# koesterlab/microphaser

Hardware: AMD Instinct MI355X
Metric: peptide-windows/s (somatic, 9-mer) (higher is better)
Workload: dtype u64

## Files before the change

### microphaser_amd/csrc/kernels.hip

```cpp
#include <hip/hip_runtime.h>

#include <algorithm>
#include <cstdlib>
#include <type_traits>

#include "kernels.hpp"

namespace mp {

#ifndef MP_KPART
#define MP_KPART -1
#endif
#define MP_IN_PART(n) (MP_KPART == -1 || MP_KPART == (n))
#define HIP_CHECK_LAUNCH() \
    do { hipError_t e_ = hipGetLastError(); if (e_ != hipSuccess) { throw_hip(e_, __FILE__, __LINE__); } } while (0)

[[noreturn]] void throw_hip(hipError_t e, const char* file, int line);

#if MP_IN_PART(0)
__global__ __launch_bounds__(256) void k0_read_variants(DeviceBatch d) {
    const uint32_t i = blockIdx.x * 256u + threadIdx.x;
    if (i >= d.n_reads) return;
    uint32_t lo = 0, hi = d.n_genes;
    while (hi - lo > 1) {
// ... 1916 lines not shown
                    tkey[idx] = 0ull;
                    tcnt[idx] = 0;
                }
                ng += uint32_t(__popcll(m));
            }
            if (ng == 0) {
                if (lane == 0) { skey[0] = 0ull; scnt[0] = 0; }
                ng = 1;
            }
            if (lane == 0) ng_lds = 0;
            __syncthreads();
            uint32_t werr = sticky_err;
            if (chunk_pos + ng > chunk_end) {
                chunk_pos = wave_claim(gcur, K2N_GROUP_CHUNK, gpart_lo);
                chunk_end = chunk_pos + K2N_GROUP_CHUNK;
            }
            const bool can_write = chunk_end <= gpart_hi;
            if (!can_write) werr |= WD_GROUP_OVERFLOW;
            if (can_write && rec_pos + ng > rec_end) {
                const uint32_t want = max(uint32_t(REC_CHUNK), ng);
                rec_pos = wave_claim(rcur, want, rpart_lo);
                rec_end = rec_pos + want;
            }
            if (can_write && rec_pos + ng > rpart_hi) sticky_err |= WD_REC_OVERFLOW;
            const uint64_t gbase = chunk_pos;
            if (can_write) {
                for (uint32_t g0 = 0; g0 < ng; g0 += 64) {
                    const uint32_t g = g0 + lane;
                    if (g < ng) {
                        const unsigned long long key = skey[g];
                        uint32_t rank = 0;
                        for (uint32_t j = 0; j < ng; j++) rank += skey[j] < key ? 1u : 0u;
                        Group G; G.hap = key; G.count = scnt[g]; G.aux = 0;
                        d.groups[gbase + rank] = G;
                    }
                    k3_enqueue(d, part, g < ng, gbase + g, win, rec_pos + g < rpart_hi ? uint32_t(rec_pos + g) : 0xFFFFFFFFu);
                }
                rec_pos += ng;
                chunk_pos += ng;
                n_groups_tx += ng;
            }
            if (lane == 0) {
                WinDyn wd;
                wd.group_off = uint32_t(gbase);
                wd.ngroups = ng;
                wd.nrows = nrows;
                wd.flags = WD_DONE | werr;
                d.win_dyn[win] = wd;
            }
            __syncthreads();
        }
    }
    if (sticky_err) atomicOr(d.err, sticky_err);
}

__device__ __forceinline__ bool is_upper(uint8_t c) { return c >= 'A' && c <= 'Z'; }
__device__ __forceinline__ uint8_t to_lower(uint8_t c) { return is_upper(c) ? uint8_t(c + 32) : c; }
__device__ __forceinline__ uint8_t to_upper(uint8_t c) { return (c >= 'a' && c <= 'z') ? uint8_t(c - 32) : c; }
__device__ __forceinline__ uint32_t rol32(uint32_t x, int n) { return (x << n) | (x >> (32 - n)); }

__device__ __forceinline__ void append_wanted(const DeviceBatch& d, bool want, uint32_t rec_slot) {
    const uint64_t m = __ballot(want);
    if (!m) return;
    const uint32_t lane = threadIdx.x & 63;
    const uint32_t leader = uint32_t(__builtin_ctzll(m));
    const uint32_t part = (blockIdx.x + blockIdx.y) & (NPART - 1);
    unsigned long long base = 0;
    if (lane == leader) base = atomicAdd(d.cursors + part * 32 + 24, (unsigned long long)__popcll(m));
    const uint64_t b0 = (uint64_t(rdlane(uint32_t(base >> 32), leader)) << 32) | rdlane(uint32_t(base), leader);
    if (want) {
        const uint64_t off = b0 + lanes_below(m, lane);
        if (off < (1ull << d.rec_part_log2)) d.want_recs[(uint64_t(part) << d.rec_part_log2) + off] = rec_slot;
        else atomicOr(d.err, WD_REC_OVERFLOW);
    }
}

constexpr int K3_THREADS = 64;
constexpr int K3_REFCAP = 36;
template <int CAP> struct K3Cfg {
    static constexpr int SLOT_BYTES = K3_REFCAP + 2 * CAP;
    static constexpr int SLOT_DW = (SLOT_BYTES / 4) | 1;
};

template <bool BUF>
struct ShaStreamT {
    uint32_t h0, h1, h2, h3, h4;
    uint64_t q;
    uint32_t nq, widx, total;
    uint32_t* blk;
    __device__ __forceinline__ void init(uint32_t* b) {
        h0 = 0x67452301u; h1 = 0xEFCDAB89u; h2 = 0x98BADCFEu; h3 = 0x10325476u; h4 = 0xC3D2E1F0u;
        q = 0; nq = 0; widx = 0; total = 0; blk = b;
    }
    __device__ void compress(uint32_t off = 0) {
        uint32_t w[16];
#pragma unroll
        for (int i = 0; i < 16; i++) w[i] = blk[off + i];
        uint32_t a = h0, b = h1, c = h2, d = h3, e = h4;
#pragma unroll
        for (int i = 0; i < 80; i++) {
            uint32_t wi;
            if (i < 16) wi = w[i];
            else {
                wi = rol32(w[(i + 13) & 15] ^ w[(i + 8) & 15] ^ w[(i + 2) & 15] ^ w[i & 15], 1);
                w[i & 15] = wi;
            }
            uint32_t f, k;
            if (i < 20) { f = (b & c) | (~b & d); k = 0x5A827999u; }
            else if (i < 40) { f = b ^ c ^ d; k = 0x6ED9EBA1u; }
            else if (i < 60) { f = (b & c) | (b & d) | (c & d); k = 0x8F1BBCDCu; }
            else { f = b ^ c ^ d; k = 0xCA62C1D6u; }
            uint32_t t = rol32(a, 5) + f + e + k + wi;
            e = d; d = c; c = rol32(b, 30); b = a; a = t;
        }
        h0 += a; h1 += b; h2 += c; h3 += d; h4 += e;
    }
    __device__ __forceinline__ void feed(uint64_t v, uint32_t n) {
        q = (q << (8 * n)) | v;
        nq += n;
        total += n;
        if (nq >= 4) {
            nq -= 4;
            blk[widx++] = uint32_t(q >> (8 * nq));
            if constexpr (!BUF) { if (widx == 16) { compress(); widx = 0; } }
            if (nq >= 4) {
                nq -= 4;
                blk[widx++] = uint32_t(q >> (8 * nq));
                if constexpr (!BUF) { if (widx == 16) { compress(); widx = 0; } }
            }
        }
    }
    __device__ void feed_dec(uint32_t v) {
        const uint32_t hi = v / 100000u, lo = v - hi * 100000u;
        auto chunk = [&](uint32_t x, bool pad) {
            uint64_t txt = 0;
            uint32_t n = 0;
            const uint32_t dg[5] = {x / 10000u, (x / 1000u) % 10u, (x / 100u) % 10u, (x / 10u) % 10u, x % 10u};
#pragma unroll
            for (int k = 0; k < 5; k++)
                if (pad || n || dg[k] || k == 4) { txt = (txt << 8) | ('0' + dg[k]); n++; }
            feed(txt, n);
        };
        if (hi) { chunk(hi, false); chunk(lo, true); }
        else chunk(lo, false);
    }
    __device__ void finish() {
        const uint32_t bits = total * 8;
        feed(0x80, 1);
        if (nq) feed(0, 4 - nq);
        while ((widx & 15) != 14) feed(0, 4);
        feed(0, 4);
        feed(bits, 4);
    }
};

__device__ __forceinline__ bool stop_codon_at(const uint8_t* s, uint32_t c, bool fwd) {
    uint8_t a = s[c], b = s[c + 1], e = s[c + 2];
    if (fwd) return a == 'T' && ((b == 'G' && e == 'A') || (b == 'A' && (e == 'G' || e == 'A')));
    return (a == 'T' && b == 'C' && e == 'A') || (a == 'C' && b == 'T' && e == 'A') || (a == 'T' && b == 'T' && e == 'A');
}

constexpr uint32_t K3B_BUF_WORDS = 48;
__device__ __forceinline__ void fill_byte_text(uint64_t* byte_text, uint32_t n_threads) {
    for (uint32_t v = threadIdx.x; v < 256; v += n_threads) {
        uint64_t txt;
        uint32_t n;
        if (v >= 100) { txt = (uint64_t('0' + v / 100) << 16) | (uint64_t('0' + (v / 10) % 10) << 8) | ('0' + v % 10); n = 3; }
        else if (v >= 10) { txt = (uint64_t('0' + v / 10) << 8) | ('0' + v % 10); n = 2; }
        else { txt = '0' + v; n = 1; }
        txt = (txt << 16) | (uint64_t(',') << 8) | ' ';
        byte_text[v] = (txt << 8) | (n + 2);
    }
}
template <int SEQ_CAP>
__device__ __forceinline__ uint64_t haplotype_id60(const DeviceBatch& d, bool active, const uint32_t* sq, uint32_t seq_len, uint32_t id_off, uint32_t id_len,
                                                   const uint32_t* idw, uint32_t id_mis, uint32_t win_sso, uint32_t* blk, const uint64_t* byte_text) {
    auto feed_message = [&](auto& sh) {
        sh.feed('[', 1);
#pragma unroll
        for (uint32_t k0 = 0; k0 < uint32_t(SEQ_CAP); k0 += 4) {
            if (k0 >= seq_len) break;
            const uint32_t dw = sq[k0 >> 2];
#pragma unroll
            for (int b = 0; b < 4; b++) {
                const uint32_t k = k0 + b;
                if (k < seq_len) {
                    const uint64_t e = byte_text[(dw >> (8 * b)) & 0xFF];
                    uint64_t txt = e >> 8;
                    uint32_t n = uint32_t(e & 0xFF);
                    if (k + 1 >= seq_len) { txt >>= 16; n -= 2; }
                    sh.feed(txt, n);
                }
            }
        }
        sh.feed(']', 1);
#pragma unroll
        for (uint32_t k = 0; k < 20; k += 4) {
            if (k < id_len) {
                const uint32_t n = min(4u, id_len - k);
                const uint32_t le = __builtin_amdgcn_alignbyte(idw[k / 4 + 1], idw[k / 4], id_mis);
                const uint32_t be = __builtin_bswap32(le) >> (8 * (4 - n));
                sh.feed(be, n);
            }
        }
        for (uint32_t k = 20; k < id_len; k += 4) {
            uint64_t txt = 0;
            const uint32_t n = min(4u, id_len - k);
            for (uint32_t c = 0; c < n; c++) txt = (txt << 8) | d.str_pool[id_off + k + c];
            sh.feed(txt, n);
        }
        sh.feed_dec(win_sso);
        sh.finish();
    };
    uint32_t o0 = 0, o1 = 0;
    const bool fits = 5 * seq_len + id_len + 20 <= K3B_BUF_WORDS * 4;
    if (__ballot(active && !fits) == 0) {
        ShaStreamT<true> sh;
        sh.init(blk);
        if (active) feed_message(sh);
        const uint32_t nblk = active ? sh.widx >> 4 : 0u;
        const uint32_t maxblk = __ballot(nblk >= 3) ? 3u : __ballot(nblk >= 2) ? 2u : __ballot(nblk >= 1) ? 1u : 0u;
        for (uint32_t bk = 0; bk < maxblk; bk++)
            if (bk < nblk) sh.compress(bk * 16);
        o0 = sh.h0; o1 = sh.h1;
    } else if (active) {
        ShaStreamT<false> sh;
        sh.init(blk);
        feed_message(sh);
        o0 = sh.h0; o1 = sh.h1;
    }
    return (uint64_t(o0) << 28) | (uint64_t(o1) >> 4);
}

template <int SEQ_CAP, int LIST, int THREADS, int K3_ITEMS>
__global__ __launch_bounds__(THREADS, LIST != 1 ? 2 : 4) void k3_window_seq(DeviceBatch d) {
    constexpr int K3_THREADS = THREADS;
    constexpr bool LIST_A = LIST != 1;
    constexpr bool STOPSCAN = LIST >= 2;
    constexpr bool WALK = LIST == 3;
    constexpr int K3_SLOT_DW = LIST_A ? ((K3Cfg<SEQ_CAP>::SLOT_DW > int(K3B_BUF_WORDS + 1) ? K3Cfg<SEQ_CAP>::SLOT_DW : int(K3B_BUF_WORDS + 1)) | 1) : K3Cfg<SEQ_CAP>::SLOT_DW;
    __shared__ uint32_t lds_slots[K3_THREADS * K3_SLOT_DW];
    __shared__ uint64_t byte_text[LIST_A ? 256 : 1];
    if constexpr (LIST_A) { fill_byte_text(byte_text, K3_THREADS); __syncthreads(); }
    const uint32_t tid = threadIdx.x;
    const uint32_t lpart = blockIdx.y;
    const uint64_t part_size = 1ull << d.group_part_log2;
    const uint64_t n_slots = min((unsigned long long)d.cursors[lpart * 32 + (LIST == 0 ? 8 : LIST == 1 ? 12 : LIST == 2 ? 20 : 28)], (unsigned long long)part_size);
    struct K3In {
        bool in_list;
        uint64_t li;
        uint64_t g;
        uint32_t w, rec_pre;
        uint64_t hap;
        WinStatic ws;
        const uint8_t* wref;
        uint32_t mis;
        uint32_t refw[K3_REFCAP / 4];
        uint32_t cp[8], ci[8];
        uint32_t id_off, id_len, id_mis;
        uint32_t idw[6];
    };
    auto load_entry = [&](K3In& I, uint64_t tile) __attribute__((always_inline)) {
        const uint64_t li = tile * K3_THREADS + tid;
        I.li = li;
        const uint64_t lidx = li < part_size ? li : part_size - 1;
        const uint64_t lpos = (uint64_t(lpart) << d.group_part_log2) + ((LIST & 1) ? part_size - 1 - lidx : lidx) + (LIST >= 2 ? d.group_cap : 0ull);
        const uint4 item = d.k3_items[lpos];
        I.g = item.x; I.w = item.y; I.rec_pre = item.z;
    };
    auto load_window = [&](K3In& I) __attribute__((always_inline)) {
        I.in_list = I.li < n_slots;
        if (!I.in_list) { I.g = 0; I.w = 0xFFFFFFFFu; I.rec_pre = 0xFFFFFFFFu; }
        if (I.w != 0xFFFFFFFFu && I.w >= d.n_wins) { I.w = 0xFFFFFFFFu; I.g = 0; }
        if (I.g >= d.group_cap) I.g = 0;
        const uint4* bp = reinterpret_cast<const uint4*>(d.win_blobs + (I.w != 0xFFFFFFFFu ? I.w : 0u));
        uint4 q[8];
#pragma unroll
        for (int k = 0; k < 8; k++) q[k] = bp[k];
        I.hap = d.groups[I.g].hap;
        static_assert(sizeof(WinStatic) == 32 && K3_REFCAP == 36, "WinBlob unpacking");
        uint32_t wsw[8] = {q[0].x, q[0].y, q[0].z, q[0].w, q[1].x, q[1].y, q[1].z, q[1].w};
        __builtin_memcpy(&I.ws, wsw, 32);
        I.refw[0] = q[2].x; I.refw[1] = q[2].y; I.refw[2] = q[2].z; I.refw[3] = q[2].w; I.refw[4] = q[3].x; I.refw[5] = q[3].y; I.refw[6] = q[3].z; I.refw[7] = q[3].w;
        I.refw[8] = q[4].x;
        const uint32_t cw[12] = {q[4].z, q[4].w, q[5].x, q[5].y, q[5].z, q[5].w, q[6].x, q[6].y, q[6].z, q[6].w, q[7].x, q[7].y};
#pragma unroll
        for (int k = 0; k < int(WINBLOB_COLS); k++) { I.cp[k] = cw[2 * k]; I.ci[k] = cw[2 * k + 1]; }
        I.id_off = q[7].z; I.id_len = q[7].w;
    };
    auto load_payload = [&](K3In& I) __attribute__((always_inline)) {
        const WinStatic& ws = I.ws;
        I.wref = d.ref_pool + ws.ref_off;
        I.mis = ws.ref_off & 3u;
        I.cp[6] = I.cp[7] = 0xFFFFFFFFu; I.ci[6] = I.ci[7] = 0;
        if (__ballot(I.w != 0xFFFFFFFFu && ws.ncols > WINBLOB_COLS)) {
            const uint32_t ncols = ws.ncols, last_c = ncols ? ncols - 1 : 0;
#pragma unroll
            for (uint32_t k = WINBLOB_COLS; k < 8; k++) { const WinCol* wc = d.win_cols + ws.col_off + min(k, last_c); I.cp[k] = wc->pos; I.ci[k] = wc->info; }
        }
    };
    auto load_id_text = [&](K3In& I) __attribute__((always_inline)) {
        I.id_mis = 0;
#pragma unroll
        for (int k = 0; k < 6; k++) I.idw[k] = 0;
        if constexpr (LIST_A) {
            const uint8_t* idp = d.str_pool + I.id_off;
            I.id_mis = uint32_t(reinterpret_cast<uintptr_t>(idp) & 3u);
#pragma unroll
            for (int k = 0; k < 6; k++) I.idw[k] = reinterpret_cast<const uint32_t*>(idp - I.id_mis)[k];
        }
    };
    uint32_t* const slot = lds_slots + tid * K3_SLOT_DW;
    uint8_t* const refb = reinterpret_cast<uint8_t*>(slot);
    uint8_t* const seq = refb + K3_REFCAP;
    uint8_t* const germ = seq + SEQ_CAP;
    auto process = [&](K3In& I) __attribute__((always_inline)) {
    const uint64_t g = I.g;
    const uint32_t w = I.w, rec_pre = I.rec_pre;
    const bool live = w != 0xFFFFFFFFu;
    const uint32_t id_off = I.id_off, id_len = I.id_len, id_mis = I.id_mis;
    const uint32_t* const idw = I.idw;
    uint32_t sumflags = 0;
    bool need_rec = false;
    uint64_t prof_set = 0;
    bool want_id = false;
    uint32_t seq_len = 0, germ_len = 0, prof_len = 0, nvar = 0, nsom = 0, first_fs = 0, first_fs_j = 0;
    uint32_t rec_sso = 0;
    if (live) {
        const WinStatic& ws = I.ws;
        rec_sso = ws.sso;
        const uint32_t vbase = ws.vbase;
        const uint64_t hap = I.hap;
        const bool is_rev = (ws.flags & WSF_REVERSE) != 0;
        const uint32_t ncols = ws.ncols;
        const uint32_t window_end = ws.sso + ws.wlen;
        const uint8_t* const wref = I.wref;
        const uint32_t mis = I.mis;
        const uint32_t* const cp = I.cp;
        const uint32_t* const ci = I.ci;
#pragma unroll
        for (int k = 0; k < K3_REFCAP / 4; k++) slot[k] = I.refw[k];
        const uint32_t staged = min(uint32_t(ws.wlen), uint32_t(K3_REFCAP) - mis);
        auto ref_at = [&](uint32_t pos) -> uint8_t {
            uint32_t k = pos - ws.sso;
            return k < staged ? refb[mis + k] : wref[k];
        };
        uint32_t i = ws.sso, j = 0, ns = 0, ngm = 0;
        bool indel = false, insertion = false, broke_flag = false;
        if (ws.flags & WSF_SIMPLE) {
#pragma unroll
            for (int k = 0; k < 8; k++) {
                const uint32_t v = __builtin_amdgcn_alignbyte(slot[k + 1], slot[k], mis);
                slot[K3_REFCAP / 4 + k] = v;
                slot[(K3_REFCAP + SEQ_CAP) / 4 + k] = v;
            }
            auto substitute = [&](uint32_t dq, uint32_t pos, uint32_t info) {
                const uint32_t off = pos - ws.sso;
                const uint8_t r = refb[mis + off];
                const uint8_t alt = uint8_t(info >> VI_ALT_SHIFT);
                const uint8_t sw = is_upper(r) ? to_lower(alt) : alt;
                seq[off] = sw;
                if (info & VI_GERMLINE) germ[off] = sw; else nsom++;
                nvar++;
                prof_set |= 1ull << (is_rev ? (ncols - 1 - dq) : dq);
            };
            const uint32_t vis = ws.need_recs >> WS_PREFIX_SHIFT;
            const uint32_t dlo = is_rev ? ncols - vis : 0u, dhi = is_rev ? ncols : vis;
#pragma unroll
            for (int k = 0; k < 8; k++)
                if (uint32_t(k) >= dlo && uint32_t(k) < dhi && ((hap >> (ncols - 1 - k)) & 1)) substitute(uint32_t(k), cp[k], ci[k]);
            for (uint32_t k = max(8u, dlo); k < dhi; k++)
                if ((hap >> (ncols - 1 - k)) & 1) { const WinCol wc = d.win_cols[ws.col_off + k]; substitute(k, wc.pos, wc.info); }
            ns = ngm = ws.wlen;
            j = vis;
            if (STOPSCAN && vis > 0 && vis < ncols) {
                const uint32_t dq_last = is_rev ? ncols - vis : vis - 1;
                const WinCol lc = d.win_cols[ws.col_off + dq_last];
                if (lc.pos + 1 == window_end && ((hap >> (ncols - 1 - dq_last)) & 1)) {
                    uint32_t cnt = 0;
                    for (uint32_t wi = vis; wi < ncols; wi++) {
                        const uint32_t dq = is_rev ? ncols - 1 - wi : wi;
                        const WinCol wc = d.win_cols[ws.col_off + dq];
                        if (wc.pos != window_end + cnt) break;
                        j = wi + 1;
                        if (!((hap >> (ncols - 1 - dq)) & 1)) break;
                        const uint32_t off = uint32_t(ws.wlen) + cnt;
                        const uint8_t r = ref_at(wc.pos);
                        const uint8_t alt = uint8_t(wc.info >> VI_ALT_SHIFT);
                        const uint8_t sw = is_upper(r) ? to_lower(alt) : alt;
                        if (off < uint32_t(SEQ_CAP)) { seq[off] = sw; germ[off] = (wc.info & VI_GERMLINE) ? sw : r; }
                        ns++; ngm++; cnt++;
                        if (!(wc.info & VI_GERMLINE)) nsom++;
                        nvar++;
                        prof_set |= 1ull << wi;
                    }
                }
            }
        } else if constexpr (!WALK) {
            atomicOr(d.err, WD_INTERNAL);
        } else {
            uint32_t pos_j = 0xFFFFFFFFu, info_j = 0, f_j = 0;
            uint32_t cpos[8], cinfo[8];
    #pragma unroll
            for (int k = 0; k < 8; k++) {
                cpos[k] = 0xFFFFFFFFu; cinfo[k] = 0;
                if (uint32_t(k) < ncols) {
                    const uint32_t dq = is_rev ? (ncols - 1 - k) : uint32_t(k);
                    if (is_rev || dq >= 8) { const WinCol* wc = d.win_cols + ws.col_off + dq; cpos[k] = wc->pos; cinfo[k] = wc->info; }
                    else { cpos[k] = cp[k]; cinfo[k] = ci[k]; }
                }
            }
            auto load_j = [&]() {
                if (j < 8) {
                    pos_j = cpos[0]; info_j = cinfo[0];
    #pragma unroll
                    for (int k = 1; k < 8; k++) if (j == uint32_t(k)) { pos_j = cpos[k]; info_j = cinfo[k]; }
                    if (j >= ncols) pos_j = 0xFFFFFFFFu;
                } else if (j < ncols) {
                    uint32_t dq = is_rev ? (ncols - 1 - j) : j;
                    const WinCol wc = d.win_cols[ws.col_off + dq];
                    pos_j = wc.pos;
                    info_j = wc.info;
                } else {
                    pos_j = 0xFFFFFFFFu;
                }
            };
            auto col_f = [&]() { return d.win_cols[ws.col_off + (is_rev ? (ncols - 1 - j) : j)].f; };
            auto push_s = [&](uint8_t c) { if (ns < SEQ_CAP) seq[ns] = c; ns++; };
            auto push_g = [&](uint8_t c) { if (ngm < SEQ_CAP) germ[ngm] = c; ngm++; };
            load_j();
            while (i < window_end) {
                while (j < ncols && i == pos_j) {
                    uint32_t fs = (info_j & VI_FS_MASK) >> VI_FS_SHIFT;
                    if (first_fs == 0 && fs) { first_fs = fs; first_fs_j = j; }
                    uint32_t dq = is_rev ? (ncols - 1 - j) : j;
                    uint32_t bit = ncols - 1 - dq;
                    if ((hap >> bit) & 1) {
// ... 4 lines not shown
                        if (kind == 0) {
                            uint8_t alt = uint8_t(info_j >> VI_ALT_SHIFT);
                            uint8_t sw = is_upper(r) ? to_lower(alt) : alt;
                            push_g(germline ? sw : r);
                            push_s(sw);
                            i += 1;
                        } else if (kind == 1) {
                            f_j = col_f();
                            uint32_t il = d.v_len[vbase + f_j] + 1;
                            const uint8_t* ins = d.ins_pool + d.v_insoff[vbase + f_j];
                            bool up = is_upper(r);
                            for (uint32_t k = 0; k < il; k++) {
                                uint8_t c = up ? to_lower(ins[k]) : to_upper(ins[k]);
                                if (germline) push_g(c);
                                push_s(c);
                            }
                            if (!germline) indel = true;
                            insertion = true;
                            i += 1;
                        } else {
                            f_j = col_f();
                            uint32_t dl = d.v_len[vbase + f_j];
                            if (is_rev && pos_j + dl - 1 >= window_end) { brk = true; }
                            else {
                                if (germline || i == window_end - 1) push_g(r);
                                else {
                                    for (uint32_t k = 0; k < dl + 1; k++) push_g(ref_at(i + k));
                                    indel = true;
                                }
                                push_s(r);
                                i += dl + 1;
                            }
                        }
                        if (brk) { broke_flag = true; break; }
                        if (!germline) nsom++;
                        nvar++;
                        prof_set |= 1ull << j;
                    }
                    j++;
                    load_j();
                }
                if (i < window_end) {
                    uint32_t stop_at = (j < ncols && pos_j > i) ? min(pos_j, window_end) : window_end;
                    for (; i < stop_at; i++) { uint8_t r = ref_at(i); push_s(r); push_g(r); }
                }
            }
        }
        seq_len = min(ns, uint32_t(SEQ_CAP));
        germ_len = min(ngm, uint32_t(SEQ_CAP));
        prof_len = j;
        uint32_t this_len = seq_len < ws.ewl ? seq_len : ws.ewl;
        uint32_t nlo = 0, nhi = seq_len;
        if (ws.splice_pos == 1) nlo = min(uint32_t(ws.splice_gap), seq_len);
        else if (ws.splice_pos == 0 && !insertion) nhi = this_len;
        bool stop = false;
        uint32_t nlen = nhi - nlo;
        if constexpr (!STOPSCAN) {
            if (!(ws.flags & WSF_NOSTOP)) atomicOr(d.err, WD_INTERNAL);
        } else if (nlen >= 3 && !(ws.flags & WSF_NOSTOP)) {
            if (!is_rev) {
                for (uint32_t c = 0; c + 3 <= nlen; c += 3)
                    if (stop_codon_at(seq + nlo, c, true)) { stop = true; break; }
            } else {
                for (int c = int(nlen) - 3; c >= 0; c -= 3)
                    if (stop_codon_at(seq + nlo, uint32_t(c), false)) { stop = true; break; }
            }
        }
        bool differs;
        if (!WALK || (ws.flags & WSF_SIMPLE)) differs = nsom > 0;
        else {
            differs = seq_len != germ_len;
            if (!differs)
                for (uint32_t k = 0; k < seq_len; k++)
                    if (seq[k] != germ[k]) { differs = true; break; }
        }
        sumflags = GS_VALID | (stop ? GS_STOP : 0) | (differs ? GS_DIFFERS : 0) | (indel ? GS_INDEL : 0) |
                   (insertion ? GS_INSERTION : 0) | (broke_flag ? GS_BROKE : 0);
        need_rec = nsom > 0 || (ws.need_recs & WS_MASK) != 0;
        want_id = need_rec && (nsom > 0 || (ws.need_recs & WS_ALL_IDS));
        if (stop && ws.splice_pos != 2 && !(ws.flags & SF_FIRST_EXON_WIN)) atomicMin(&d.tx_first_stop[ws.tx], w);
    }
    uint32_t recidx = 0;
    {
        uint32_t sqr[2 * SEQ_CAP / 4];
#pragma unroll
        for (int k = 0; k < 2 * SEQ_CAP / 4; k++) sqr[k] = slot[K3_REFCAP / 4 + k];
        const bool has_slot = live && rec_pre != 0xFFFFFFFFu;
        const bool hash = has_slot && need_rec && want_id;
        uint64_t id60 = 0;
        if constexpr (LIST_A) {
            id60 = haplotype_id60<SEQ_CAP>(d, hash && !d.timing_skip_ids, sqr, seq_len, id_off, id_len, idw, id_mis, rec_sso, slot, byte_text);
            const uint64_t hm = __ballot(hash);
            if (hm && (tid & 63u) == uint32_t(__builtin_ctzll(hm))) atomicAdd(d.cursors + ((blockIdx.x + blockIdx.y) & (NPART - 1)) * 32 + 24, (unsigned long long)__popcll(hm));
        } else if (hash) {
            atomicOr(d.err, WD_REC_OVERFLOW);
        }
        if (has_slot) {
            uint32_t* out = reinterpret_cast<uint32_t*>(d.recs + uint64_t(rec_pre) * d.rec_stride);
            if (need_rec) {
                uint4* const out4 = reinterpret_cast<uint4*>(out);
                out4[0] = make_uint4(uint32_t(prof_set), uint32_t(prof_set >> 32), uint32_t(id60), uint32_t(id60 >> 32));
                out4[1] = make_uint4(seq_len | (germ_len << 8) | (prof_len << 16) | (nvar << 24), nsom | (first_fs << 8) | (first_fs_j << 16), w, want_id ? 1u : 0u);
#pragma unroll
                for (int k = 0; k < SEQ_CAP / 16; k++) {
                    if (uint32_t(16 * k) < seq_len) out4[2 + k] = make_uint4(sqr[4 * k], sqr[4 * k + 1], sqr[4 * k + 2], sqr[4 * k + 3]);
                    if (uint32_t(16 * k) < germ_len) {
                        constexpr int G = SEQ_CAP / 16;
                        out4[2 + G + k] = make_uint4(sqr[4 * (G + k)], sqr[4 * (G + k) + 1], sqr[4 * (G + k) + 2], sqr[4 * (G + k) + 3]);
                    }
                }
                sumflags |= GS_HAS_REC | ((LIST_A && want_id) ? uint32_t(GS_ID_VALID) : 0u);
                recidx = rec_pre;
            } else {
                out[7] = 0;
            }
        } else if (live && need_rec) {
            atomicOr(d.err, WD_REC_OVERFLOW);
        }
    }
    if (live) {
        GroupSum gs;
        gs.flags = sumflags;
        gs.rec = recidx;
        d.gsum[g] = gs;
    }
    };
    for (uint64_t tile0 = uint64_t(blockIdx.x) * K3_ITEMS;; tile0 += uint64_t(gridDim.x) * K3_ITEMS) {
        static_assert(K3_ITEMS == 1 || K3_ITEMS == 2, "entries per lane");
        K3In in0, in1;
        load_entry(in0, tile0);
        if constexpr (K3_ITEMS == 2) load_entry(in1, tile0 + 1);
        if (tile0 * K3_THREADS >= n_slots) break;
        if (pass_overflowed(d)) return;
        load_window(in0);
        if constexpr (K3_ITEMS == 2) load_window(in1);
        load_payload(in0);
        if constexpr (K3_ITEMS == 2) load_payload(in1);
        load_id_text(in0);
        if constexpr (K3_ITEMS == 2) load_id_text(in1);
        process(in0);
        if constexpr (K3_ITEMS == 2) process(in1);
    }
}

template <int SEQ_CAP>
__device__ __forceinline__ uint32_t k3n_one(const DeviceBatch& d, uint32_t* lds_slots, uint64_t g, uint32_t item_win, uint32_t item_rec, bool valid,
                                            uint32_t& recidx) {
    constexpr int K3_SLOT_DW = K3Cfg<SEQ_CAP>::SLOT_DW;
    const uint32_t tid = threadIdx.x;
    recidx = 0;
    uint32_t* slot = lds_slots + tid * K3_SLOT_DW;
    uint8_t* refb = reinterpret_cast<uint8_t*>(slot);
    uint8_t* seq = refb + K3_REFCAP;
    uint32_t* germ_dw = slot + (K3_REFCAP + SEQ_CAP) / 4;
    const uint32_t w = valid ? item_win : 0xFFFFFFFFu;
    if (w == 0xFFFFFFFFu) return 0;
    const WinStatic ws = d.wins[w];
    const uint32_t vbase = ws.vbase;
    const Group G = d.groups[g];
    const uint64_t hap = G.hap;
    const uint32_t nrows = d.win_dyn[w].nrows;
    const bool freq_one = G.count != 0 && G.count == nrows;
    const bool is_rev = (ws.flags & WSF_REVERSE) != 0;
    const uint32_t ncols = ws.ncols;
    uint32_t window_end = ws.sso + ws.wlen;
    const uint8_t* wref = d.ref_pool + ws.ref_off;
    const uint32_t mis = uint32_t(reinterpret_cast<uintptr_t>(wref) & 3u);
    {
        const uint32_t* src = reinterpret_cast<const uint32_t*>(wref - mis);
        const uint32_t ndw = (mis + ws.wlen + 3) >> 2;
        for (uint32_t k = 0; k < ndw && k < K3_REFCAP / 4; k++) slot[k] = src[k];
    }
    const uint32_t staged = min(uint32_t(ws.wlen), uint32_t(K3_REFCAP) - mis);
    auto ref_at = [&](uint32_t pos) -> uint8_t {
        uint32_t k = pos - ws.sso;
        return k < staged ? refb[mis + k] : wref[k];
    };
    auto col = [&](uint32_t j) { return d.win_cols[ws.col_off + (is_rev ? (ncols - 1 - j) : j)]; };
    uint32_t i = ws.sso, j = 0, ns = 0, prof_len = 0, nvar = 0, nsom = 0;
    uint64_t prof_set = 0, prof_som = 0;
    bool insertion = false;
    auto push_s = [&](uint8_t c) { if (ns < SEQ_CAP) seq[ns] = c; ns++; };
    if (ncols == 0) {
        for (; i < window_end; i++) push_s(ref_at(i));
    } else {
        WinCol cj = col(0);
        while (i < window_end) {
            while (j < ncols && i == cj.pos) {
                if (freq_one && !(cj.info & VI_GERMLINE)) {
                    j++; prof_len++;
                    if (j < ncols) cj = col(j);
                    continue;
                }
                if ((hap >> j) & 1) {
                    if (j + 1 < ncols) {
                        const WinCol nx = col(j + 1);
                        if (nx.pos == i) { j++; cj = nx; }
                    }
                    const uint32_t kind = cj.info & VI_KIND_MASK;
                    const uint8_t r = ref_at(i);
                    if (kind == 0) {
                        const uint8_t alt = uint8_t(cj.info >> VI_ALT_SHIFT);
                        push_s(is_upper(r) ? to_lower(alt) : alt);
                        i += 1;
                    } else if (kind == 1) {
                        const uint32_t il = d.v_len[vbase + cj.f] + 1;
                        const uint8_t* ins = d.ins_pool + d.v_insoff[vbase + cj.f];
                        const bool up = is_upper(r);
                        for (uint32_t k = 0; k < il; k++) push_s(up ? to_lower(ins[k]) : to_upper(ins[k]));
                        insertion = true;
                        i += 1;
                    } else {
                        const uint32_t dl = d.v_len[vbase + cj.f];
                        push_s(r);
                        i += dl + 1;
                        window_end += dl + 1;
                    }
                    if (prof_len < 64) {
                        prof_set |= 1ull << prof_len;
                        if (!(cj.info & VI_GERMLINE)) prof_som |= 1ull << prof_len;
                    }
                    if (!(cj.info & VI_GERMLINE)) nsom++;
                    nvar++;
                }
                prof_len++;
                j++;
                if (j < ncols) cj = col(j);
            }
            push_s(ref_at(i));
            i += 1;
        }
    }
    const uint32_t seq_len = min(ns, uint32_t(SEQ_CAP));
    uint32_t nlo = 0, nhi = seq_len;
    if (ws.splice_pos == 1) nlo = min(uint32_t(ws.splice_gap), seq_len);
    else if (ws.splice_pos == 0 && !insertion) nhi = min(seq_len, uint32_t(ws.ewl));
    bool stop = false;
    if (nhi - nlo >= 3) stop = is_rev ? stop_codon_at(seq, nhi - 3, false) : stop_codon_at(seq, nlo, true);
    const bool skipped = stop && ws.splice_pos != 2;
    uint32_t sumflags = GS_VALID | (stop ? GS_STOP : 0) | (insertion ? GS_INSERTION : 0) | (ns > uint32_t(SEQ_CAP) ? uint32_t(GS_BROKE) : 0u);
    const uint32_t slot_idx = item_rec;
    if (slot_idx != 0xFFFFFFFFu) {
        uint32_t* out = reinterpret_cast<uint32_t*>(d.recs + uint64_t(slot_idx) * d.rec_stride);
        germ_dw[0] = uint32_t(prof_som); germ_dw[1] = uint32_t(prof_som >> 32);
        out[0] = uint32_t(prof_set); out[1] = uint32_t(prof_set >> 32);
        out[2] = ws.sso; out[3] = ws.tx;
        out[4] = seq_len | (0u << 8) | (min(prof_len, 255u) << 16) | (min(nvar, 255u) << 24);
        out[5] = min(nsom, 255u);
        out[6] = w;
        out[7] = skipped ? 0u : 1u;
        const uint32_t* sq = slot + K3_REFCAP / 4;
#pragma unroll
        for (int k = 0; k < 2 * SEQ_CAP / 4; k++) out[8 + k] = sq[k];
        sumflags |= GS_HAS_REC | (skipped ? 0u : uint32_t(GS_ID_VALID));
        recidx = slot_idx;
    } else {
        atomicOr(d.err, WD_REC_OVERFLOW);
    }
    GroupSum gs;
    gs.flags = sumflags;
    gs.rec = recidx;
    d.gsum[g] = gs;
    return sumflags;
}
template <int SEQ_CAP>
__global__ __launch_bounds__(K3_THREADS) void k3_window_seq_normal(DeviceBatch d) {
    __shared__ uint32_t lds_slots[K3_THREADS * K3Cfg<SEQ_CAP>::SLOT_DW];
    const uint32_t lpart = blockIdx.y;
    if (pass_overflowed(d)) return;
    const uint64_t n_slots = min((unsigned long long)d.cursors[lpart * 32 + 8], 1ull << d.group_part_log2);
    for (uint64_t tile = blockIdx.x; tile * K3_THREADS < n_slots; tile += gridDim.x) {
        const uint64_t li = tile * K3_THREADS + threadIdx.x;
        const uint64_t lpos = (uint64_t(lpart) << d.group_part_log2) + li;
        const uint4 item = d.k3_items[li < n_slots ? lpos : (uint64_t(lpart) << d.group_part_log2)];
        uint32_t recidx;
        const uint32_t sumflags = k3n_one<SEQ_CAP>(d, lds_slots, item.x, item.y, item.z, li < n_slots, recidx);
        append_wanted(d, (sumflags & GS_ID_VALID) != 0, recidx);
    }
}

constexpr uint32_t K3B_THREADS = 192;
template <int SEQ_CAP>
__global__ __launch_bounds__(K3B_THREADS) void k3b_haplotype_ids(DeviceBatch d) {
    __shared__ uint32_t lds_blk[K3B_THREADS * (K3B_BUF_WORDS + 1)];
    __shared__ uint64_t byte_text[256];
    fill_byte_text(byte_text, K3B_THREADS);
    __syncthreads();
    const uint32_t wp = blockIdx.y;
    if (pass_overflowed(d)) return;
    const uint64_t n_recs = min((unsigned long long)d.cursors[wp * 32 + 24], 1ull << d.rec_part_log2);
    for (uint64_t tile = blockIdx.x; tile * K3B_THREADS < n_recs; tile += gridDim.x) {
    const uint64_t li = tile * K3B_THREADS + threadIdx.x;
    const bool active = li < n_recs;
    const uint64_t r = d.want_recs[(uint64_t(wp) << d.rec_part_log2) + (active ? li : 0)];
    uint32_t* rec = reinterpret_cast<uint32_t*>(d.recs + r * d.rec_stride);
    const uint4* rec4 = reinterpret_cast<const uint4*>(rec);
    const uint4 h0 = rec4[0], h1 = rec4[1];
    uint32_t sq[SEQ_CAP / 4];
#pragma unroll
    for (int k = 0; k < SEQ_CAP / 16; k++) { const uint4 v = rec4[2 + k]; sq[4 * k] = v.x; sq[4 * k + 1] = v.y; sq[4 * k + 2] = v.z; sq[4 * k + 3] = v.w; }
    const uint32_t seq_len = h1.x & 0xFF, win_sso = h0.z;
    const TxDev T = d.tx[active ? h0.w : 0];
    const uint8_t* idp = d.str_pool + T.id_off;
    const uint32_t id_mis = uint32_t(reinterpret_cast<uintptr_t>(idp) & 3u);
    uint32_t idw[6];
#pragma unroll
    for (int k = 0; k < 6; k++) idw[k] = reinterpret_cast<const uint32_t*>(idp - id_mis)[k];
    const uint64_t id60 = haplotype_id60<SEQ_CAP>(d, active, sq, seq_len, T.id_off, T.id_len, idw, id_mis, win_sso,
                                                  lds_blk + threadIdx.x * (K3B_BUF_WORDS + 1), byte_text);
    if (active) {
        rec[2] = uint32_t(id60);
        rec[3] = uint32_t(id60 >> 32);
    }
    }
}

#if MP_IN_PART(0)
void launch_k1_pileup_bits(const DeviceBatch& d, hipStream_t stream) {
    if (d.n_reads == 0) return;
    dim3 grid(uint32_t((uint64_t(d.n_reads) * K1_LANES + 255) / 256)), block(256);
    switch (d.mask_words) {
        case 1: hipLaunchKernelGGL(k1_pileup_bits<1>, grid, block, 0, stream, d); break;
        case 2: hipLaunchKernelGGL(k1_pileup_bits<2>, grid, block, 0, stream, d); break;
        case 3: case 4: {
            DeviceBatch d4 = d;
            if (d.mask_words == 3) throw_hip(hipErrorInvalidValue, __FILE__, __LINE__);
            hipLaunchKernelGGL(k1_pileup_bits<4>, grid, block, 0, stream, d4);
            break;
        }
        default: throw_hip(hipErrorInvalidValue, __FILE__, __LINE__);
    }
    HIP_CHECK_LAUNCH();
}

#endif
#if MP_IN_PART(1)
void launch_k2_window_replay(const DeviceBatch& d, int rows_per_lane, hipStream_t stream) {
    if (d.n_segs == 0) return;
    dim3 grid(d.n_segs), block(64);
    if (d.normal) {
#define K2N_CASE(R) case R: if (d.normal_large) hipLaunchKernelGGL((k2n_window_replay<R, 512, 2048>), grid, block, 0, stream, d); \
                            else hipLaunchKernelGGL((k2n_window_replay<R, 128, 512>), grid, block, 0, stream, d); break;
        switch (rows_per_lane) {
            K2N_CASE(1) K2N_CASE(2) K2N_CASE(4) K2N_CASE(8) K2N_CASE(16)
            default: throw_hip(hipErrorInvalidValue, __FILE__, __LINE__);
        }
#undef K2N_CASE
        HIP_CHECK_LAUNCH();
        return;
    }
    switch (rows_per_lane) {
        case 1: hipLaunchKernelGGL(k2_window_replay<1>, grid, block, 0, stream, d); break;
        case 2: hipLaunchKernelGGL(k2_window_replay<2>, grid, block, 0, stream, d); break;
        case 4: hipLaunchKernelGGL(k2_window_replay<4>, grid, block, 0, stream, d); break;
        case 8: hipLaunchKernelGGL(k2_window_replay<8>, grid, block, 0, stream, d); break;
        case 16: hipLaunchKernelGGL(k2_window_replay<16>, grid, block, 0, stream, d); break;
        default: throw_hip(hipErrorInvalidValue, __FILE__, __LINE__);
    }
    HIP_CHECK_LAUNCH();
}

#endif
#if MP_IN_PART(0)
void launch_k2_admission(const DeviceBatch& d, hipStream_t stream) {
    if (!d.n_adm) return;
    const dim3 grid(uint32_t((d.n_adm + 63) / 64)), block(64);
    if (d.mask_words == 1) hipLaunchKernelGGL(k2a_admission_flat<1>, grid, block, 0, stream, d);
    else if (d.mask_words == 2) hipLaunchKernelGGL(k2a_admission_flat<2>, grid, block, 0, stream, d);
    else throw_hip(hipErrorInvalidValue, __FILE__, __LINE__);
    HIP_CHECK_LAUNCH();
}
#endif
#if MP_IN_PART(2)
template <int W>
static void launch_k2w_multi(const DeviceBatch& d, hipStream_t stream) {
    dim3 grid(d.n_wchunks_m), block(64);
    switch (d.rows_per_lane_w) {
        case 1: hipLaunchKernelGGL((k2w_window_rows_multi<1, W>), grid, block, 0, stream, d); break;
        case 2: hipLaunchKernelGGL((k2w_window_rows_multi<2, W>), grid, block, 0, stream, d); break;
        case 4: hipLaunchKernelGGL((k2w_window_rows_multi<4, W>), grid, block, 0, stream, d); break;
        case 8: hipLaunchKernelGGL((k2w_window_rows_multi<8, W>), grid, block, 0, stream, d); break;
        default: throw_hip(hipErrorInvalidValue, __FILE__, __LINE__);
    }
}
void launch_k2_window_rows(const DeviceBatch& d, hipStream_t stream) {
    if (d.n_wchunks) {
        hipLaunchKernelGGL(k2w_window_rows, dim3((d.n_wchunks + K2W_ITEMS - 1) / K2W_ITEMS), dim3(64), 0, stream, d);
        HIP_CHECK_LAUNCH();
    }
    if (d.n_wchunks_m) {
        if (d.mask_words == 1) launch_k2w_multi<1>(d, stream);
        else if (d.mask_words == 2) launch_k2w_multi<2>(d, stream);
// ... 104 lines not shown
```

Measured before the change: 2.512 billion.

## Stream SHA-1 haplotype IDs block-by-block with wave-uniform compress loop

Replaces the two SHA-1 paths (a 48-word LDS-buffered path and a per-lane streaming fallback) with one streaming loop. Each iteration fills a 16-word block in LDS and compresses it, and the loop repeats under a wave ballot until every lane has finished its message. The slot layout is reordered so the sequence bytes are read straight from LDS instead of copied into registers, and the byte-to-text table shrinks to 32-bit entries. This is meant to cut LDS footprint and register pressure and raise occupancy, at the cost of more complex per-block padding logic and possible extra divergent compress iterations.

```diff
diff --git a/microphaser_amd/csrc/kernels.hip b/microphaser_amd/csrc/kernels.hip
--- a/microphaser_amd/csrc/kernels.hip
+++ b/microphaser_amd/csrc/kernels.hip
@@ -2022,20 +2022,17 @@
     static constexpr int SLOT_DW = (SLOT_BYTES / 4) | 1;
 };
 
-template <bool BUF>
-struct ShaStreamT {
+struct Sha1Lane {
     uint32_t h0, h1, h2, h3, h4;
-    uint64_t q;
-    uint32_t nq, widx, total;
     uint32_t* blk;
     __device__ __forceinline__ void init(uint32_t* b) {
         h0 = 0x67452301u; h1 = 0xEFCDAB89u; h2 = 0x98BADCFEu; h3 = 0x10325476u; h4 = 0xC3D2E1F0u;
-        q = 0; nq = 0; widx = 0; total = 0; blk = b;
-    }
-    __device__ void compress(uint32_t off = 0) {
+        blk = b;
+    }
+    __device__ void compress() {
         uint32_t w[16];
 #pragma unroll
-        for (int i = 0; i < 16; i++) w[i] = blk[off + i];
+        for (int i = 0; i < 16; i++) w[i] = blk[i];
         uint32_t a = h0, b = h1, c = h2, d = h3, e = h4;
 #pragma unroll
         for (int i = 0; i < 80; i++) {
@@ -2055,43 +2052,6 @@
         }
         h0 += a; h1 += b; h2 += c; h3 += d; h4 += e;
     }
-    __device__ __forceinline__ void feed(uint64_t v, uint32_t n) {
-        q = (q << (8 * n)) | v;
-        nq += n;
-        total += n;
-        if (nq >= 4) {
-            nq -= 4;
-            blk[widx++] = uint32_t(q >> (8 * nq));
-            if constexpr (!BUF) { if (widx == 16) { compress(); widx = 0; } }
-            if (nq >= 4) {
-                nq -= 4;
-                blk[widx++] = uint32_t(q >> (8 * nq));
-                if constexpr (!BUF) { if (widx == 16) { compress(); widx = 0; } }
-            }
-        }
-    }
-    __device__ void feed_dec(uint32_t v) {
-        const uint32_t hi = v / 100000u, lo = v - hi * 100000u;
-        auto chunk = [&](uint32_t x, bool pad) {
-            uint64_t txt = 0;
-            uint32_t n = 0;
-            const uint32_t dg[5] = {x / 10000u, (x / 1000u) % 10u, (x / 100u) % 10u, (x / 10u) % 10u, x % 10u};
-#pragma unroll
-            for (int k = 0; k < 5; k++)
-                if (pad || n || dg[k] || k == 4) { txt = (txt << 8) | ('0' + dg[k]); n++; }
-            feed(txt, n);
-        };
-        if (hi) { chunk(hi, false); chunk(lo, true); }
-        else chunk(lo, false);
-    }
-    __device__ void finish() {
-        const uint32_t bits = total * 8;
-        feed(0x80, 1);
-        if (nq) feed(0, 4 - nq);
-        while ((widx & 15) != 14) feed(0, 4);
-        feed(0, 4);
-        feed(bits, 4);
-    }
 };
 
 __device__ __forceinline__ bool stop_codon_at(const uint8_t* s, uint32_t c, bool fwd) {
@@ -2100,87 +2060,113 @@
     return (a == 'T' && b == 'C' && e == 'A') || (a == 'C' && b == 'T' && e == 'A') || (a == 'T' && b == 'T' && e == 'A');
 }
 
-constexpr uint32_t K3B_BUF_WORDS = 48;
-__device__ __forceinline__ void fill_byte_text(uint64_t* byte_text, uint32_t n_threads) {
+__device__ __forceinline__ void fill_byte_text(uint32_t* byte_text, uint32_t n_threads) {
     for (uint32_t v = threadIdx.x; v < 256; v += n_threads) {
-        uint64_t txt;
-        uint32_t n;
-        if (v >= 100) { txt = (uint64_t('0' + v / 100) << 16) | (uint64_t('0' + (v / 10) % 10) << 8) | ('0' + v % 10); n = 3; }
-        else if (v >= 10) { txt = (uint64_t('0' + v / 10) << 8) | ('0' + v % 10); n = 2; }
+        uint32_t txt, n;
+        if (v >= 100) { txt = (uint32_t('0' + v / 100) << 16) | (uint32_t('0' + (v / 10) % 10) << 8) | ('0' + v % 10); n = 3; }
+        else if (v >= 10) { txt = (uint32_t('0' + v / 10) << 8) | ('0' + v % 10); n = 2; }
         else { txt = '0' + v; n = 1; }
-        txt = (txt << 16) | (uint64_t(',') << 8) | ' ';
-        byte_text[v] = (txt << 8) | (n + 2);
+        byte_text[v] = (txt << 8) | n;
     }
 }
 template <int SEQ_CAP>
-__device__ __forceinline__ uint64_t haplotype_id60(const DeviceBatch& d, bool active, const uint32_t* sq, uint32_t seq_len, uint32_t id_off, uint32_t id_len,
-                                                   const uint32_t* idw, uint32_t id_mis, uint32_t win_sso, uint32_t* blk, const uint64_t* byte_text) {
-    auto feed_message = [&](auto& sh) {
-        sh.feed('[', 1);
-#pragma unroll
-        for (uint32_t k0 = 0; k0 < uint32_t(SEQ_CAP); k0 += 4) {
-            if (k0 >= seq_len) break;
-            const uint32_t dw = sq[k0 >> 2];
-#pragma unroll
-            for (int b = 0; b < 4; b++) {
-                const uint32_t k = k0 + b;
-                if (k < seq_len) {
-                    const uint64_t e = byte_text[(dw >> (8 * b)) & 0xFF];
-                    uint64_t txt = e >> 8;
-                    uint32_t n = uint32_t(e & 0xFF);
-                    if (k + 1 >= seq_len) { txt >>= 16; n -= 2; }
-                    sh.feed(txt, n);
-                }
-            }
-        }
-        sh.feed(']', 1);
-#pragma unroll
-        for (uint32_t k = 0; k < 20; k += 4) {
-            if (k < id_len) {
-                const uint32_t n = min(4u, id_len - k);
-                const uint32_t le = __builtin_amdgcn_alignbyte(idw[k / 4 + 1], idw[k / 4], id_mis);
-                const uint32_t be = __builtin_bswap32(le) >> (8 * (4 - n));
-                sh.feed(be, n);
-            }
-        }
-        for (uint32_t k = 20; k < id_len; k += 4) {
-            uint64_t txt = 0;
-            const uint32_t n = min(4u, id_len - k);
-            for (uint32_t c = 0; c < n; c++) txt = (txt << 8) | d.str_pool[id_off + k + c];
-            sh.feed(txt, n);
-        }
-        sh.feed_dec(win_sso);
-        sh.finish();
-    };
-    uint32_t o0 = 0, o1 = 0;
-    const bool fits = 5 * seq_len + id_len + 20 <= K3B_BUF_WORDS * 4;
-    if (__ballot(active && !fits) == 0) {
-        ShaStreamT<true> sh;
-        sh.init(blk);
-        if (active) feed_message(sh);
-        const uint32_t nblk = active ? sh.widx >> 4 : 0u;
-        const uint32_t maxblk = __ballot(nblk >= 3) ? 3u : __ballot(nblk >= 2) ? 2u : __ballot(nblk >= 1) ? 1u : 0u;
-        for (uint32_t bk = 0; bk < maxblk; bk++)
-            if (bk < nblk) sh.compress(bk * 16);
-        o0 = sh.h0; o1 = sh.h1;
-    } else if (active) {
-        ShaStreamT<false> sh;
-        sh.init(blk);
-        feed_message(sh);
-        o0 = sh.h0; o1 = sh.h1;
-    }
-    return (uint64_t(o0) << 28) | (uint64_t(o1) >> 4);
+__device__ __forceinline__ uint64_t haplotype_id60(const DeviceBatch& d, bool active, const uint8_t* seq, uint32_t seq_len, uint32_t id_off, uint32_t id_len,
+                                                   const uint32_t* idw, uint32_t id_mis, uint32_t win_sso, uint32_t* blk, const uint32_t* byte_text) {
+    Sha1Lane sh;
+    sh.init(blk);
+    uint64_t q = '[';
+    uint32_t nq = 1, widx = 0, k = 0;
+    uint32_t nwords = 0xFFFFFFFFu;
+    uint32_t e = seq_len ? byte_text[seq[0]] : 0u;
+    bool live = active;
+    for (uint32_t lo = 0; __ballot(live); lo += 16) {
+        if (!live) continue;
+        const uint32_t hi = lo + 16;
+        if (k < seq_len) {
+            if (nq >= 4) { nq -= 4; blk[widx++ - lo] = uint32_t(q >> (8 * nq)); }
+            while (k < seq_len && widx < hi) {
+                uint64_t txt = (uint64_t(e >> 8) << 16) | 0x2C20u;
+                uint32_t n = (e & 0xFF) + 2;
+                k++;
+                if (k < seq_len) e = byte_text[seq[k]];
+                else { txt >>= 16; n -= 2; }
+                q = (q << (8 * n)) | txt;
+                nq += n;
+                if (nq >= 4) {
+                    nq -= 4;
+                    blk[widx++ - lo] = uint32_t(q >> (8 * nq));
+                    if (nq >= 4 && widx < hi) { nq -= 4; blk[widx++ - lo] = uint32_t(q >> (8 * nq)); }
+                }
+            }
+        }
+        if (k >= seq_len) {
+            uint64_t tq = q;
+            uint32_t tnq = nq, tw = widx;
+            auto put = [&](uint32_t v) { if (tw - lo < 16u) blk[tw - lo] = v; tw++; };
+            auto feed = [&](uint64_t v, uint32_t n) {
+                tq = (tq << (8 * n)) | v;
+                tnq += n;
+                if (tnq >= 4) {
+                    tnq -= 4;
+                    put(uint32_t(tq >> (8 * tnq)));
+                    if (tnq >= 4) { tnq -= 4; put(uint32_t(tq >> (8 * tnq))); }
+                }
+            };
+            feed(']', 1);
+#pragma unroll
+            for (uint32_t c = 0; c < 20; c += 4) {
+                if (c < id_len) {
+                    const uint32_t n = min(4u, id_len - c);
+                    const uint32_t le = __builtin_amdgcn_alignbyte(idw[c / 4 + 1], idw[c / 4], id_mis);
+                    const uint32_t be = __builtin_bswap32(le) >> (8 * (4 - n));
+                    feed(be, n);
+                }
+            }
+            for (uint32_t c = 20; c < id_len; c += 4) {
+                uint64_t txt = 0;
+                const uint32_t n = min(4u, id_len - c);
+                for (uint32_t x = 0; x < n; x++) txt = (txt << 8) | d.str_pool[id_off + c + x];
+                feed(txt, n);
+            }
+            {
+                const uint32_t dhi = win_sso / 100000u, dlo = win_sso - dhi * 100000u;
+                auto chunk = [&](uint32_t x, bool pad) {
+                    uint64_t txt = 0;
+                    uint32_t n = 0;
+                    const uint32_t dg[5] = {x / 10000u, (x / 1000u) % 10u, (x / 100u) % 10u, (x / 10u) % 10u, x % 10u};
+#pragma unroll
+                    for (int j = 0; j < 5; j++)
+                        if (pad || n || dg[j] || j == 4) { txt = (txt << 8) | ('0' + dg[j]); n++; }
+                    feed(txt, n);
+                };
+                if (dhi) { chunk(dhi, false); chunk(dlo, true); }
+                else chunk(dlo, false);
+            }
+            const uint32_t bits = (4 * tw + tnq) * 8;
+            feed(0x80, 1);
+            if (tnq) feed(0, 4 - tnq);
+            nwords = (tw + 2 + 15) & ~15u;
+#pragma unroll
+            for (uint32_t i = 0; i < 16; i++)
+                if (lo + i >= tw && lo + i < nwords) blk[i] = lo + i + 1 == nwords ? bits : 0u;
+        }
+        sh.compress();
+        live = nwords > hi;
+    }
+    return (uint64_t(sh.h0) << 28) | (uint64_t(sh.h1) >> 4);
 }
 
 template <int SEQ_CAP, int LIST, int THREADS, int K3_ITEMS>
-__global__ __launch_bounds__(THREADS, LIST != 1 ? 2 : 4) void k3_window_seq(DeviceBatch d) {
+__global__ __launch_bounds__(THREADS, LIST >= 2 ? 2 : 4) void k3_window_seq(DeviceBatch d) {
     constexpr int K3_THREADS = THREADS;
     constexpr bool LIST_A = LIST != 1;
     constexpr bool STOPSCAN = LIST >= 2;
     constexpr bool WALK = LIST == 3;
-    constexpr int K3_SLOT_DW = LIST_A ? ((K3Cfg<SEQ_CAP>::SLOT_DW > int(K3B_BUF_WORDS + 1) ? K3Cfg<SEQ_CAP>::SLOT_DW : int(K3B_BUF_WORDS + 1)) | 1) : K3Cfg<SEQ_CAP>::SLOT_DW;
+    constexpr int K3_SLOT_DW = K3Cfg<SEQ_CAP>::SLOT_DW;
+    constexpr int SEQ_DW = 0, REF_DW = SEQ_CAP / 4, GERM_DW = (SEQ_CAP + K3_REFCAP) / 4;
+    static_assert(K3_SLOT_DW - REF_DW >= 16 && SEQ_CAP % 16 == 0, "slot layout");
     __shared__ uint32_t lds_slots[K3_THREADS * K3_SLOT_DW];
-    __shared__ uint64_t byte_text[LIST_A ? 256 : 1];
+    __shared__ uint32_t byte_text[LIST_A ? 256 : 1];
     if constexpr (LIST_A) { fill_byte_text(byte_text, K3_THREADS); __syncthreads(); }
     const uint32_t tid = threadIdx.x;
     const uint32_t lpart = blockIdx.y;
@@ -2251,9 +2237,9 @@
         }
     };
     uint32_t* const slot = lds_slots + tid * K3_SLOT_DW;
-    uint8_t* const refb = reinterpret_cast<uint8_t*>(slot);
-    uint8_t* const seq = refb + K3_REFCAP;
-    uint8_t* const germ = seq + SEQ_CAP;
+    uint8_t* const seq = reinterpret_cast<uint8_t*>(slot + SEQ_DW);
+    uint8_t* const refb = reinterpret_cast<uint8_t*>(slot + REF_DW);
+    uint8_t* const germ = reinterpret_cast<uint8_t*>(slot + GERM_DW);
     auto process = [&](K3In& I) __attribute__((always_inline)) {
     const uint64_t g = I.g;
     const uint32_t w = I.w, rec_pre = I.rec_pre;
@@ -2279,7 +2265,7 @@
         const uint32_t* const cp = I.cp;
         const uint32_t* const ci = I.ci;
 #pragma unroll
-        for (int k = 0; k < K3_REFCAP / 4; k++) slot[k] = I.refw[k];
+        for (int k = 0; k < K3_REFCAP / 4; k++) slot[REF_DW + k] = I.refw[k];
         const uint32_t staged = min(uint32_t(ws.wlen), uint32_t(K3_REFCAP) - mis);
         auto ref_at = [&](uint32_t pos) -> uint8_t {
             uint32_t k = pos - ws.sso;
@@ -2290,9 +2276,9 @@
         if (ws.flags & WSF_SIMPLE) {
 #pragma unroll
             for (int k = 0; k < 8; k++) {
-                const uint32_t v = __builtin_amdgcn_alignbyte(slot[k + 1], slot[k], mis);
-                slot[K3_REFCAP / 4 + k] = v;
-                slot[(K3_REFCAP + SEQ_CAP) / 4 + k] = v;
+                const uint32_t v = __builtin_amdgcn_alignbyte(slot[REF_DW + k + 1], slot[REF_DW + k], mis);
+                slot[SEQ_DW + k] = v;
+                slot[GERM_DW + k] = v;
             }
             auto substitute = [&](uint32_t dq, uint32_t pos, uint32_t info) {
                 const uint32_t off = pos - ws.sso;
@@ -2463,41 +2449,36 @@
     }
     uint32_t recidx = 0;
     {
-        uint32_t sqr[2 * SEQ_CAP / 4];
-#pragma unroll
-        for (int k = 0; k < 2 * SEQ_CAP / 4; k++) sqr[k] = slot[K3_REFCAP / 4 + k];
         const bool has_slot = live && rec_pre != 0xFFFFFFFFu;
         const bool hash = has_slot && need_rec && want_id;
+        uint4* const out4 = reinterpret_cast<uint4*>(d.recs + uint64_t(has_slot ? rec_pre : 0u) * d.rec_stride);
+        if (has_slot) {
+            if (need_rec) {
+                out4[1] = make_uint4(seq_len | (germ_len << 8) | (prof_len << 16) | (nvar << 24), nsom | (first_fs << 8) | (first_fs_j << 16), w, want_id ? 1u : 0u);
+#pragma unroll
+                for (int k = 0; k < SEQ_CAP / 16; k++) {
+                    if (uint32_t(16 * k) < seq_len)
+                        out4[2 + k] = make_uint4(slot[SEQ_DW + 4 * k], slot[SEQ_DW + 4 * k + 1], slot[SEQ_DW + 4 * k + 2], slot[SEQ_DW + 4 * k + 3]);
+                    if (uint32_t(16 * k) < germ_len)
+                        out4[2 + SEQ_CAP / 16 + k] = make_uint4(slot[GERM_DW + 4 * k], slot[GERM_DW + 4 * k + 1], slot[GERM_DW + 4 * k + 2], slot[GERM_DW + 4 * k + 3]);
+                }
+                sumflags |= GS_HAS_REC | ((LIST_A && want_id) ? uint32_t(GS_ID_VALID) : 0u);
+                recidx = rec_pre;
+            } else {
+                reinterpret_cast<uint32_t*>(out4)[7] = 0;
+            }
+        } else if (live && need_rec) {
+            atomicOr(d.err, WD_REC_OVERFLOW);
+        }
         uint64_t id60 = 0;
         if constexpr (LIST_A) {
-            id60 = haplotype_id60<SEQ_CAP>(d, hash && !d.timing_skip_ids, sqr, seq_len, id_off, id_len, idw, id_mis, rec_sso, slot, byte_text);
+            id60 = haplotype_id60<SEQ_CAP>(d, hash && !d.timing_skip_ids, seq, seq_len, id_off, id_len, idw, id_mis, rec_sso, slot + REF_DW, byte_text);
             const uint64_t hm = __ballot(hash);
             if (hm && (tid & 63u) == uint32_t(__builtin_ctzll(hm))) atomicAdd(d.cursors + ((blockIdx.x + blockIdx.y) & (NPART - 1)) * 32 + 24, (unsigned long long)__popcll(hm));
         } else if (hash) {
             atomicOr(d.err, WD_REC_OVERFLOW);
         }
-        if (has_slot) {
-            uint32_t* out = reinterpret_cast<uint32_t*>(d.recs + uint64_t(rec_pre) * d.rec_stride);
-            if (need_rec) {
-                uint4* const out4 = reinterpret_cast<uint4*>(out);
-                out4[0] = make_uint4(uint32_t(prof_set), uint32_t(prof_set >> 32), uint32_t(id60), uint32_t(id60 >> 32));
-                out4[1] = make_uint4(seq_len | (germ_len << 8) | (prof_len << 16) | (nvar << 24), nsom | (first_fs << 8) | (first_fs_j << 16), w, want_id ? 1u : 0u);
-#pragma unroll
-                for (int k = 0; k < SEQ_CAP / 16; k++) {
-                    if (uint32_t(16 * k) < seq_len) out4[2 + k] = make_uint4(sqr[4 * k], sqr[4 * k + 1], sqr[4 * k + 2], sqr[4 * k + 3]);
-                    if (uint32_t(16 * k) < germ_len) {
-                        constexpr int G = SEQ_CAP / 16;
-                        out4[2 + G + k] = make_uint4(sqr[4 * (G + k)], sqr[4 * (G + k) + 1], sqr[4 * (G + k) + 2], sqr[4 * (G + k) + 3]);
-                    }
-                }
-                sumflags |= GS_HAS_REC | ((LIST_A && want_id) ? uint32_t(GS_ID_VALID) : 0u);
-                recidx = rec_pre;
-            } else {
-                out[7] = 0;
-            }
-        } else if (live && need_rec) {
-            atomicOr(d.err, WD_REC_OVERFLOW);
-        }
+        if (has_slot && need_rec) out4[0] = make_uint4(uint32_t(prof_set), uint32_t(prof_set >> 32), uint32_t(id60), uint32_t(id60 >> 32));
     }
     if (live) {
         GroupSum gs;
@@ -2663,10 +2644,12 @@
 constexpr uint32_t K3B_THREADS = 192;
 template <int SEQ_CAP>
 __global__ __launch_bounds__(K3B_THREADS) void k3b_haplotype_ids(DeviceBatch d) {
-    __shared__ uint32_t lds_blk[K3B_THREADS * (K3B_BUF_WORDS + 1)];
-    __shared__ uint64_t byte_text[256];
+    constexpr uint32_t SLOT_DW = (SEQ_CAP / 4 + 16) | 1;
+    __shared__ uint32_t lds_slots[K3B_THREADS * SLOT_DW];
+    __shared__ uint32_t byte_text[256];
     fill_byte_text(byte_text, K3B_THREADS);
     __syncthreads();
+    uint32_t* const slot = lds_slots + threadIdx.x * SLOT_DW;
     const uint32_t wp = blockIdx.y;
     if (pass_overflowed(d)) return;
     const uint64_t n_recs = min((unsigned long long)d.cursors[wp * 32 + 24], 1ull << d.rec_part_log2);
@@ -2677,18 +2660,22 @@
     uint32_t* rec = reinterpret_cast<uint32_t*>(d.recs + r * d.rec_stride);
     const uint4* rec4 = reinterpret_cast<const uint4*>(rec);
     const uint4 h0 = rec4[0], h1 = rec4[1];
-    uint32_t sq[SEQ_CAP / 4];
-#pragma unroll
-    for (int k = 0; k < SEQ_CAP / 16; k++) { const uint4 v = rec4[2 + k]; sq[4 * k] = v.x; sq[4 * k + 1] = v.y; sq[4 * k + 2] = v.z; sq[4 * k + 3] = v.w; }
-    const uint32_t seq_len = h1.x & 0xFF, win_sso = h0.z;
+    const uint32_t seq_len = min(h1.x & 0xFFu, uint32_t(SEQ_CAP)), win_sso = h0.z;
+#pragma unroll
+    for (int k = 0; k < SEQ_CAP / 16; k++) {
+        if (uint32_t(16 * k) < seq_len) {
+            const uint4 v = rec4[2 + k];
+            slot[4 * k] = v.x; slot[4 * k + 1] = v.y; slot[4 * k + 2] = v.z; slot[4 * k + 3] = v.w;
+        }
+    }
     const TxDev T = d.tx[active ? h0.w : 0];
     const uint8_t* idp = d.str_pool + T.id_off;
     const uint32_t id_mis = uint32_t(reinterpret_cast<uintptr_t>(idp) & 3u);
     uint32_t idw[6];
 #pragma unroll
     for (int k = 0; k < 6; k++) idw[k] = reinterpret_cast<const uint32_t*>(idp - id_mis)[k];
-    const uint64_t id60 = haplotype_id60<SEQ_CAP>(d, active, sq, seq_len, T.id_off, T.id_len, idw, id_mis, win_sso,
-                                                  lds_blk + threadIdx.x * (K3B_BUF_WORDS + 1), byte_text);
+    const uint64_t id60 = haplotype_id60<SEQ_CAP>(d, active, reinterpret_cast<const uint8_t*>(slot), seq_len, T.id_off, T.id_len, idw, id_mis, win_sso,
+                                                  slot + SEQ_CAP / 4, byte_text);
     if (active) {
         rec[2] = uint32_t(id60);
         rec[3] = uint32_t(id60 >> 32);
```

Result: no change. 2.538 billion (median of 6 runs) (+1.0%).
